# ytabatabaee/fastconsensus

Measured on AMD Instinct MI355X. Metric: consensus wall time + partition·edges/sec, LFR 1M nodes n_p=64, 1/2/4/8 GPUs, higher is better.
Workload: dtype int32

## Files before the change

fastconsensus_amd/csrc/cd_rl.hip:

```cpp
#include <hipcub/hipcub.hpp>

#include <chrono>

#include "fc_ctx.h"
#include "fc_device.h"

namespace fc {

template <class T> void exclusive_scan(Ctx& c, const T* in, T* out, int64_t n);

namespace {

constexpr int RTB = 64;
constexpr int DM = 64;
constexpr int VPWMAX = 8;
constexpr int RL_CHUNK = 16;
constexpr int RL_MAX_REPLICAS = 16384;
#ifndef FC_RL_SPLIT
#define FC_RL_SPLIT 30
#endif
#ifndef FC_LPA_TIES
#define FC_LPA_TIES 1
#endif

constexpr int32_t DONE = -1;
constexpr int NSH = 16;
constexpr int RF = 8;
constexpr double DQ_SCALE = 1099511627776.0;
constexpr int HWSLOTS = 1024;
constexpr int HTB = 256;
constexpr int HEAVY_GRID = 2048;
constexpr int SLOW_GRID = 256;
constexpr int LTB = 256;
constexpr int LPER = 8;
constexpr int NCLS = 6;
__host__ __device__ __forceinline__ int rl_class(int d) {
    return d <= 16 ? 0 : d <= 24 ? 1 : d <= 32 ? 2 : d <= 48 ? 3 : d <= DM ? 4 : 5;
}

struct RL {
    int64_t N, S, PN;
    int chunk;
    uint32_t perm_n;
    int B;
    int n_r, rbase, LG, VPW, banks, ldT;
    int lgs;
    uint32_t iter;
    uint64_t seed;
    const int64_t* rowptr;
    const int32_t* col;
    const int32_t* cw;
    const int4* vrec;
    const int64_t* kdeg;
    int64_t M2;
    int unitw;
    int wbits;
    const int32_t* colw;
    int32_t* lab;
    int32_t* tot;
    int32_t* dec;
    int64_t* slow;
    int32_t* slow_cnt;
    int4* list;
    uint64_t* lmask;
    uint64_t* vmask;
    int32_t* boff;
    int32_t* cursor;
    int32_t* voff;
    int32_t* vcursor;
    int64_t* vlist;
    uint64_t* aff;
    uint64_t* mvf;
    int32_t* active;
    int32_t* track;
    int prune, lm, track_div;
    unsigned long long* red;
    unsigned long long* sacc;
    int32_t* hscratch;
    int64_t hslots;
    double min_dq;
    int hybrid;
    const int32_t* acnt;
    int dense_div;
};
__device__ __forceinline__ bool rl_sparse(const RL& a, int r) {
    return a.hybrid && a.active[r] && a.prune && a.track[a.n_r + r] && (int64_t)a.dense_div * a.acnt[r] < a.N;
}

__device__ __forceinline__ Perm rl_perm(const RL& a, int sweep) {
    Perm P = make_perm(a.perm_n, stream_key(a.seed, SHARED_RG, a.iter, (uint32_t)sweep, 1));
    if (a.chunk) P.off = stream_key(a.seed, SHARED_RG, a.iter, (uint32_t)sweep, 3) & (RL_CHUNK - 1);
    return P;
}
__device__ __forceinline__ uint32_t rl_bucket(const RL& a, const Perm& P, uint32_t v) {
    uint32_t pos;
    if (!a.chunk) pos = perm_invert(P, v);
    else {
        const uint32_t w = v + P.off;
        pos = perm_invert(P, w / RL_CHUNK) * RL_CHUNK + w % RL_CHUNK;
    }
    return pos / (uint32_t)a.S;
}
__device__ __forceinline__ unsigned long long* rl_red(const RL& a, int r, int f) {
    return a.red + ((size_t)r * NSH + (blockIdx.x & (NSH - 1))) * RF + f;
}
__device__ __forceinline__ bool rl_better(long long s1, uint32_t h1, int32_t c1, long long s2, uint32_t h2,
                                          int32_t c2) {
    if (s1 != s2) return s1 > s2;
    if (h1 != h2) return h1 > h2;
    return c1 < c2;
}
__device__ __forceinline__ int32_t ld_off(const int32_t* base, uint32_t i) {
    return *reinterpret_cast<const int32_t*>(reinterpret_cast<const char*>(base) + (i << 2));
}
__device__ __forceinline__ int wave_max(int x) {
#pragma unroll
    for (int off = 32; off > 0; off >>= 1) x = max(x, __shfl_xor(x, off));
    return x;
}
__device__ __forceinline__ void wsync() {
    __builtin_amdgcn_wave_barrier();
    asm volatile("" ::: "memory");
}

__device__ __forceinline__ void rl_tie_flag(const RL& a, int rr, int32_t v) {
    atomicOr((unsigned long long*)&a.aff[(int64_t)(rr >> 6) * a.N + v], 1ull << (rr & 63));
}

__global__ void k_rl_init(int64_t N, int ldT, const int64_t* kdeg, int32_t* lab, int32_t* tot) {
    const int64_t i = (int64_t)blockIdx.x * blockDim.x + threadIdx.x;
    if (i >= N * ldT) return;
    const int64_t v = i / ldT;
    lab[i] = (int32_t)v;
    if (tot) tot[i] = (int32_t)kdeg[v];
}
__global__ __launch_bounds__(256) void k_rl_export(int64_t N, int n_r, int ldT, const int32_t* labT, const int32_t* sinv,
                                                   int32_t* lab) {
    __shared__ int32_t t[64][65];
    __shared__ int32_t sv[64];
    const int64_t s0 = (int64_t)blockIdx.x * 64;
    const int r0 = blockIdx.y * 64;
    const int tx = threadIdx.x & 63, ty = threadIdx.x >> 6;
    if (ty == 0) sv[tx] = s0 + tx < N ? (sinv ? sinv[s0 + tx] : (int32_t)(s0 + tx)) : -1;
    __syncthreads();
    for (int ss = ty; ss < 64; ss += 4) {
        const int32_t v = sv[ss];
        const int r = r0 + tx;
        if (v >= 0 && r < n_r) t[ss][tx] = labT[(int64_t)v * ldT + r];
    }
    __syncthreads();
    for (int rr = ty; rr < 64; rr += 4) {
        const int r = r0 + rr;
        if (r < n_r && s0 + tx < N) lab[(int64_t)r * N + s0 + tx] = t[tx][rr];
    }
}

__global__ __launch_bounds__(LTB) void k_rl_list_count(RL a, int sweep, int listed, int32_t* bcnt, int32_t* vcnt) {
    extern __shared__ unsigned long long s_dyn[];
    uint64_t* s_act = (uint64_t*)s_dyn;
    uint64_t* s_flt = s_act + a.banks;
    int* s_b = (int*)(s_flt + a.banks);
    int* s_v = s_b + a.B * NCLS;
    for (int k = threadIdx.x; k < a.B * NCLS; k += LTB) { s_b[k] = 0; s_v[k] = 0; }
    for (int b = threadIdx.x; b < a.banks; b += LTB) { s_act[b] = 0; s_flt[b] = 0; }
    __syncthreads();
    for (int r = threadIdx.x; r < a.n_r; r += LTB) {
        if (!a.active[r]) continue;
        atomicOr((unsigned long long*)&s_act[r >> 6], 1ull << (r & 63));
        if (a.prune && a.track[a.n_r + r]) atomicOr((unsigned long long*)&s_flt[r >> 6], 1ull << (r & 63));
    }
    __syncthreads();
    if (a.hybrid && listed) {
        bool any = false;
        for (int r = 0; r < a.n_r && !any; ++r) any = rl_sparse(a, r);
        if (any) return;
    }
    const Perm P = rl_perm(a, sweep);
    const int64_t v0 = (int64_t)blockIdx.x * LTB * LPER + threadIdx.x;
#pragma unroll
    for (int i = 0; i < LPER; ++i) {
        const int64_t v = v0 + (int64_t)i * LTB;
        if (v >= a.N) break;
        int nv = 0;
        for (int b = 0; b < a.banks; ++b) {
            uint64_t f = a.aff[(int64_t)b * a.N + v];
            if (listed && f) a.aff[(int64_t)b * a.N + v] = 0;
            const uint64_t m = s_act[b] & (~s_flt[b] | f);
            a.vmask[v * a.banks + b] = m;
            nv += __popcll(m);
        }
        if (nv) {
            const int sg = rl_bucket(a, P, (uint32_t)v) * NCLS + rl_class(a.vrec[v].y);
            atomicAdd(&s_b[sg], 1);
            atomicAdd(&s_v[sg], nv);
        }
    }
    __syncthreads();
    for (int k = threadIdx.x; k < a.B * NCLS; k += LTB) {
        if (s_b[k]) atomicAdd(&bcnt[k], s_b[k]);
        if (s_v[k]) atomicAdd(&vcnt[k], s_v[k]);
    }
}
__global__ void k_rl_list_plan(int nseg, int32_t* bcnt, int32_t* boff, int32_t* cursor, int32_t* vcnt,
                               int32_t* voff, int32_t* vcursor, const int32_t* n_active) {
    if (threadIdx.x != 0) return;
    int32_t acc = 0, vacc = 0;
    for (int k = 0; k < nseg; ++k) {
        boff[k] = acc; cursor[k] = acc; acc += bcnt[k];
        voff[k] = vacc; vcursor[k] = vacc; vacc += vcnt[k];
        bcnt[k] = 0; vcnt[k] = 0;
    }
    boff[nseg] = acc;
    voff[nseg] = vacc;
    voff[nseg + 1] = n_active[0];
    voff[nseg + 2] = n_active[1];
}
__global__ __launch_bounds__(LTB) void k_rl_visits_count(RL a, int64_t n_entries, int32_t* nv) {
    const int64_t e = (int64_t)blockIdx.x * LTB + threadIdx.x;
    if (e >= n_entries) return;
    int c = 0;
    for (int b = 0; b < a.banks; ++b) c += __popcll(a.lmask[e * a.banks + b]);
    nv[e] = c;
}
__global__ __launch_bounds__(LTB) void k_rl_visits_fill(RL a, int64_t n_entries, const int32_t* vpos) {
    const int64_t e = (int64_t)blockIdx.x * LTB + threadIdx.x;
    if (e >= n_entries) return;
    int64_t pos = vpos[e];
    for (int b = 0; b < a.banks; ++b) {
        uint64_t m = a.lmask[e * a.banks + b];
        while (m) {
            const int bit = __ffsll((unsigned long long)m) - 1;
            m &= m - 1;
            a.vlist[pos++] = (e << 14) | (int64_t)(b * 64 + bit);
        }
    }
}

__global__ __launch_bounds__(LTB) void k_rl_list_fill(RL a, int sweep) {
    extern __shared__ int s_lb[];
    int* s_cnt = s_lb;
    int* s_base = s_lb + a.B * NCLS;
    for (int k = threadIdx.x; k < a.B * NCLS; k += LTB) s_cnt[k] = 0;
    __syncthreads();
    const Perm P = rl_perm(a, sweep);
    int bk[LPER], loc[LPER];
    const int64_t v0 = (int64_t)blockIdx.x * LTB * LPER + threadIdx.x;
#pragma unroll
    for (int i = 0; i < LPER; ++i) {
        const int64_t v = v0 + (int64_t)i * LTB;
        bk[i] = -1;
        if (v >= a.N) continue;
        bool any = false;
        for (int b = 0; b < a.banks; ++b) any |= a.vmask[v * a.banks + b] != 0;
        if (!any) continue;
        bk[i] = (int)rl_bucket(a, P, (uint32_t)v) * NCLS + rl_class(a.vrec[v].y);
        loc[i] = atomicAdd(&s_cnt[bk[i]], 1);
    }
    __syncthreads();
    for (int k = threadIdx.x; k < a.B * NCLS; k += LTB) s_base[k] = s_cnt[k] ? atomicAdd(&a.cursor[k], s_cnt[k]) : 0;
    __syncthreads();
#pragma unroll
    for (int i = 0; i < LPER; ++i) {
        if (bk[i] < 0) continue;
        const int64_t v = v0 + (int64_t)i * LTB;
        const int64_t e = s_base[bk[i]] + loc[i];
        const int4 vr = a.vrec[v];
        a.list[e] = make_int4((int32_t)v, vr.x, vr.y, vr.z);
        for (int b = 0; b < a.banks; ++b) a.lmask[e * a.banks + b] = a.vmask[v * a.banks + b];
    }
}

struct Unit {
    int64_t e;
    int bank, s, rl, r;
    bool valid;
};
__device__ __forceinline__ Unit rl_unit(const RL& a, int64_t e0, int64_t e1, int64_t w) {
    Unit u;
    const int lane = threadIdx.x & 63;
    u.s = lane >> a.lgs;
    u.rl = lane & (a.LG - 1);
    if (a.banks == 1) { u.e = e0 + (w << (6 - a.lgs)) + u.s; u.bank = 0; }
    else { u.e = e0 + w / a.banks; u.bank = (int)(w % a.banks); }
    u.r = u.bank * 64 + u.rl;
    u.valid = u.e < e1 && u.s < a.VPW;
    return u;
}
__device__ __forceinline__ int64_t rl_items(const RL& a, int64_t n) {
    return a.banks == 1 ? (n + a.VPW - 1) / a.VPW : n * a.banks;
}

struct Hdr {
    int32_t v;
    uint64_t msk;
    int64_t rb;
    int d, kvi, ds, rr;
    bool on, heavy, work;
};
struct Rec {
    int4 e;
    uint64_t msk;
};
__device__ __forceinline__ Rec rl_fetch(const RL& a, const Unit& u) {
    Rec r;
    r.e = make_int4(-1, 0, 0, 0);
    r.msk = 0;
    if (u.valid) {
        r.e = a.list[u.e];
        r.msk = a.lmask[u.e * a.banks + u.bank];
    }
    return r;
}
__device__ __forceinline__ Hdr rl_header(const RL& a, const Unit& u, const Rec& rec) {
    Hdr h;
    h.rr = u.bank * 64 + u.rl;
    h.v = rec.e.x;
    h.msk = rec.msk;
    h.rb = (int64_t)(uint32_t)rec.e.y;
    h.d = rec.e.z;
    h.kvi = rec.e.w;
    h.on = u.valid && h.rr < a.n_r && ((h.msk >> u.rl) & 1ull);
    h.heavy = u.valid && h.d > DM;
    h.work = h.on && !h.heavy && h.d > 0;
    h.ds = (u.valid && !h.heavy && h.msk) ? h.d : 0;
    return h;
}

template <int K>
__device__ __forceinline__ void oem_sort(int32_t (&x)[K]) {
#pragma unroll
    for (int p = 1; p < K; p <<= 1)
#pragma unroll
        for (int k = p; k >= 1; k >>= 1)
#pragma unroll
            for (int j = k % p; j + k < K; j += 2 * k)
#pragma unroll
                for (int i = 0; i < k; ++i)
                    if ((i + j) / (2 * p) == (i + j + k) / (2 * p) && i + j + k < K) {
                        const int32_t a = x[i + j], b = x[i + j + k];
                        x[i + j] = min(a, b);
                        x[i + j + k] = max(a, b);
                    }
}

constexpr int WM_WIDE = 0, WM_UNIT = 1, WM_W8 = 2;
#ifndef FC_RL_SB
#define FC_RL_SB 16
#endif
constexpr int SB = FC_RL_SB;
#ifndef FC_RL_LPA_OWN
#define FC_RL_LPA_OWN 1
#endif
template <bool LOUV, int K, int WM>
__device__ __forceinline__ int32_t rl_runs(const RL& a, const Hdr& h, int sweep, int32_t (&x)[K], int32_t own,
                                           long long kown, int32_t tot_own, uint32_t home, unsigned long long& c_dq,
                                           uint32_t& c_unst, uint32_t& c_cand, bool& slow_out) {
    constexpr bool UNITW = WM == WM_UNIT;
    const uint32_t rr = (uint32_t)h.rr, ldT = (uint32_t)a.ldT;
    const int wb = UNITW ? 0 : a.wbits;
    const int32_t wm = (1 << wb) - 1;
    const bool wk = h.work;
    oem_sort<K>(x);
    int vm = INT_MIN;
    {
        int acc = 0;
        int32_t kl = (int32_t)kown;
#pragma unroll
        for (int q = 0; q < K; ++q) {
            const int32_t l = x[q] >> wb;
            const int w = UNITW ? 1 : (x[q] & wm);
            acc = (q > 0 && l == (x[q - 1] >> wb)) ? acc + w : w;
            const bool end = x[q] >= 0 && (q == K - 1 || (x[q + 1] >> wb) != l);
            vm = end ? max(vm, acc) : vm;
            if (!LOUV && !FC_RL_LPA_OWN) kl = (end && l == own) ? acc : kl;
        }
        if (!LOUV && !FC_RL_LPA_OWN) kown = kl;
        if (!LOUV && FC_RL_LPA_OWN) vm = max(vm, (int)kown);
    }
    bool hope = true;
    if (LOUV) hope = wk && ((long long)vm - kown) * a.M2 + (long long)h.kvi * ((long long)tot_own - h.kvi) > 0;
    uint32_t cm_lo = 0, cm_hi = 0;
    if (hope) {
        int acc = 0;
#pragma unroll
        for (int q = 0; q < K; ++q) {
            const int32_t l = x[q] >> wb;
            const int w = UNITW ? 1 : (x[q] & wm);
            acc = (q > 0 && l == (x[q - 1] >> wb)) ? acc + w : w;
            const bool cand = x[q] >= 0 && (q == K - 1 || (x[q + 1] >> wb) != l) && acc == vm;
            if (q < 32) cm_lo |= (uint32_t)cand << (q & 31);
            else cm_hi |= (uint32_t)cand << (q & 31);
        }
    }
    const bool own_cand = !LOUV && FC_RL_LPA_OWN && wk && kown > 0 && kown == (long long)vm;
    const int ncand = __popc(cm_lo) + __popc(cm_hi) + (own_cand ? 1 : 0);
    if (wk) c_cand += (uint32_t)ncand;
    const uint32_t tvh = hash32(stream_key(a.seed, (uint32_t)(a.rbase + h.rr), a.iter, (uint32_t)sweep, 2) ^ (uint32_t)h.v);
    int32_t dcs = -1;
    if (LOUV) {
        const long long kv = h.kvi;
        uint64_t bkey = ~0ull;
#pragma unroll
        for (int c0 = 0; c0 < K; c0 += SB) {
            const uint32_t bits = ((c0 < 32 ? cm_lo : cm_hi) >> (c0 & 31)) & ((1u << SB) - 1u);
            if (__ballot(bits != 0) == 0) continue;
            int32_t tq[SB];
#pragma unroll
            for (int i = 0; i < SB; ++i) {
                if (c0 + i >= K) break;
                const bool b = (bits >> i) & 1u;
                tq[i] = ld_off(a.tot, b ? (uint32_t)(x[c0 + i] >> wb) * ldT + rr : home);
            }
#pragma unroll
            for (int i = 0; i < SB; ++i) {
                if (c0 + i >= K) break;
                const bool b = (bits >> i) & 1u;
                const uint32_t hh = hash32(tvh ^ (uint32_t)(x[c0 + i] >> wb));
                const uint64_t key = ((uint64_t)(kv ? (uint32_t)tq[i] : 0u) << 32) | (uint32_t)~hh;
                bkey = (b && key < bkey) ? key : bkey;
            }
        }
        long long best_s = LLONG_MIN;
        uint32_t best_h = 0;
        int32_t best_c = INT_MAX;
        if (ncand != 0) {
            best_h = ~(uint32_t)bkey;
            best_c = (int32_t)(hash32_inv(best_h) ^ tvh);
            best_s = (long long)vm * a.M2 - kv * (long long)(uint32_t)(bkey >> 32);
        }
        slow_out = wk && ncand != 0 && (long long)(vm - 1) * a.M2 >= best_s;
        if (wk && ncand != 0 && !slow_out) {
            const long long G = best_s - kown * a.M2 + kv * ((long long)tot_own - kv);
            if (G > 0) {
                const double dqd = (double)G * 2.0 / ((double)a.M2 * (double)a.M2);
                c_dq += (unsigned long long)llrint(dqd * DQ_SCALE);
                dcs = best_c;
            }
        }
    } else {
        uint32_t best_h = 0;
        int32_t best_c = -1;
#pragma unroll
        for (int q = 0; q < K; ++q) {
            const bool b = ((q < 32 ? cm_lo : cm_hi) >> (q & 31)) & 1u;
            const uint32_t hh = hash32(tvh ^ (uint32_t)x[q]);
            const bool take = b && (best_c < 0 || hh > best_h);
            best_h = take ? hh : best_h;
            best_c = take ? x[q] : best_c;
        }
        if (own_cand) {
            const uint32_t hh = hash32(tvh ^ (uint32_t)own);
            if (best_c < 0 || hh > best_h) { best_h = hh; best_c = own; }
        }
        if (wk && ncand != 0) {
            c_unst += (kown != (long long)vm) ? 1 : 0;
            dcs = best_c != own ? best_c : -1;
        }
    }
    return dcs;
}

template <bool LOUV, int K, int WM>
__device__ __forceinline__ int32_t rl_sorted(const RL& a, const Hdr& h, int sweep, unsigned long long& c_dq,
                                             uint32_t& c_unst, uint32_t& c_cand, bool& slow_out) {
    constexpr bool UNITW = WM == WM_UNIT;
    slow_out = false;
    const uint32_t rr = (uint32_t)h.rr, ldT = (uint32_t)a.ldT;
    const int wb = UNITW ? 0 : a.wbits;
    const int32_t wm = (1 << wb) - 1;
    const bool wk = h.work;
    const uint32_t home = (h.v >= 0 ? (uint32_t)h.v : 0u) * ldT + rr;
    const int32_t own0 = ld_off(a.lab, home);
    const int32_t own = wk ? own0 : -1;
    const int dsw = wk ? h.ds : 0;
    int32_t x[K];
#pragma unroll
    for (int j = 0; j < K; ++j)
        x[j] = ld_off(WM == WM_W8 ? a.colw : a.col, (uint32_t)h.rb + (uint32_t)(j < dsw ? j : 0));
    int32_t tot_own = 0;
    if (LOUV) {
        const int32_t t0 = ld_off(a.tot, wk ? (uint32_t)own * ldT + rr : home);
        tot_own = wk ? t0 : 0;
    }
    long long kown = 0;
    if constexpr (UNITW) {
#pragma unroll
        for (int j = 0; j < K; ++j) {
            const int32_t lj = ld_off(a.lab, j < dsw ? (uint32_t)x[j] * ldT + rr : home);
            x[j] = j < dsw ? lj : -1;
        }
        if (LOUV || FC_RL_LPA_OWN) {
            int ko = 0;
#pragma unroll
            for (int j = 0; j < K; ++j) {
                const bool mine = x[j] == own && x[j] >= 0;
                ko += mine ? 1 : 0;
                x[j] = mine ? -1 : x[j];
            }
            kown = ko;
        }
    } else if constexpr (WM == WM_W8) {
        uint32_t wpk[(K + 3) / 4];
#pragma unroll
        for (int i = 0; i < (K + 3) / 4; ++i) wpk[i] = 0;
#pragma unroll
        for (int j = 0; j < K; ++j) wpk[j >> 2] |= (uint32_t)(x[j] & wm) << (8 * (j & 3));
#pragma unroll
        for (int j = 0; j < K; ++j) {
            const int32_t lj = ld_off(a.lab, j < dsw ? (uint32_t)(x[j] >> wb) * ldT + rr : home);
            x[j] = j < dsw ? lj : -1;
        }
        int ko = 0;
#pragma unroll
        for (int j = 0; j < K; ++j) {
            const int32_t wj = (int32_t)((wpk[j >> 2] >> (8 * (j & 3))) & 0xffu);
            const bool mine = LOUV && x[j] == own && x[j] >= 0;
            ko += mine ? wj : 0;
            x[j] = (mine || x[j] < 0) ? -1 : ((x[j] << wb) | wj);
        }
        kown = ko;
    } else {
        int32_t wv[K];
#pragma unroll
        for (int j = 0; j < K; ++j) {
            const int32_t wj = ld_off(a.cw, (uint32_t)h.rb + (uint32_t)(j < dsw ? j : 0));
            wv[j] = j < dsw ? wj : 0;
        }
#pragma unroll
        for (int j = 0; j < K; ++j) {
            const int32_t lj = ld_off(a.lab, j < dsw ? (uint32_t)x[j] * ldT + rr : home);
            x[j] = j < dsw ? lj : -1;
        }
        int ko = 0;
#pragma unroll
        for (int j = 0; j < K; ++j) {
            const bool mine = LOUV && x[j] == own && x[j] >= 0;
            ko += mine ? wv[j] : 0;
            x[j] = (mine || x[j] < 0) ? -1 : ((x[j] << wb) | wv[j]);
        }
        kown = ko;
    }
    if (LOUV) {
        const long long kvl = h.kvi;
        const bool settled = !wk || (kvl - 2 * kown) * a.M2 + kvl * ((long long)tot_own - kvl) <= 0;
        if (__ballot(!settled) == 0) return -1;
    } else if (FC_RL_LPA_OWN) {
        const bool settled = !wk || 2 * kown > (long long)dsw;
        if (__ballot(!settled) == 0) {
            if (wk) c_cand += 1u;
            return -1;
        }
    }
    constexpr int KN = (K == 32 && (FC_RL_SPLIT & 8)) ? 16 : (K == 64 && (FC_RL_SPLIT & 16)) ? 48 : K;
    if constexpr (KN < K) {
        if (__builtin_amdgcn_readfirstlane(wave_max(dsw)) <= KN) {
            int32_t y[KN];
#pragma unroll
            for (int j = 0; j < KN; ++j) y[j] = x[j];
            return rl_runs<LOUV, KN, WM>(a, h, sweep, y, own, kown, tot_own, home, c_dq, c_unst, c_cand, slow_out);
        }
    }
    return rl_runs<LOUV, K, WM>(a, h, sweep, x, own, kown, tot_own, home, c_dq, c_unst, c_cand, slow_out);
}

struct RowPre {
    int32_t col;
    int32_t w;
    int32_t own;
};
__device__ __forceinline__ Rec rl_fetch_u(const RL& a, const Unit& u) {
    Rec r = rl_fetch(a, u);
    r.e.x = __builtin_amdgcn_readfirstlane(r.e.x);
    r.e.y = __builtin_amdgcn_readfirstlane(r.e.y);
    r.e.z = __builtin_amdgcn_readfirstlane(r.e.z);
    r.e.w = __builtin_amdgcn_readfirstlane(r.e.w);
    r.msk = ((uint64_t)(uint32_t)__builtin_amdgcn_readfirstlane((int32_t)(r.msk >> 32)) << 32) |
            (uint32_t)__builtin_amdgcn_readfirstlane((int32_t)r.msk);
    return r;
}
template <int WM>
__device__ __forceinline__ RowPre rl_row_pre(const RL& a, const Unit& u, const Rec& r) {
    RowPre p;
    p.col = 0; p.w = 0; p.own = 0;
    const uint32_t lane = threadIdx.x & 63;
    if (r.e.x >= 0) {
        const int d = r.e.z;
        if (d > 0 && d <= DM) {
            const uint32_t j = lane < (uint32_t)d ? lane : 0u;
            p.col = ld_off(WM == WM_W8 ? a.colw : a.col, (uint32_t)r.e.y + j);
            if (WM == WM_WIDE) p.w = ld_off(a.cw, (uint32_t)r.e.y + j);
        }
        p.own = ld_off(a.lab, (uint32_t)r.e.x * (uint32_t)a.ldT + (uint32_t)(u.bank * 64) + lane);
    }
    return p;
}
template <bool LOUV, int K, int WM>
__device__ __forceinline__ int32_t rl_sorted_u1(const RL& a, const Hdr& h, int sweep, const RowPre& pre,
                                                unsigned long long& c_dq, uint32_t& c_unst, uint32_t& c_cand,
                                                bool& slow_out) {
    constexpr bool UNITW = WM == WM_UNIT;
    slow_out = false;
    const uint32_t rr = (uint32_t)h.rr, ldT = (uint32_t)a.ldT;
    const int wb = UNITW ? 0 : a.wbits;
    const int32_t wm = (1 << wb) - 1;
    const bool wk = h.work;
    const int ds = h.ds;
    if (ds == 0) return -1;
    const uint32_t home = (uint32_t)h.v * ldT + rr;
    const int32_t own = wk ? pre.own : -1;
    int32_t x[K];
#pragma unroll
    for (int j = 0; j < K; ++j) {
        const int32_t cj = __builtin_amdgcn_readlane(pre.col, j);
        const uint32_t id = (uint32_t)(WM == WM_W8 ? (cj >> wb) : cj);
        x[j] = ld_off(a.lab, id * ldT + rr);
    }
    int32_t tot_own = 0;
    if (LOUV) {
        const int32_t t0 = ld_off(a.tot, wk ? (uint32_t)own * ldT + rr : home);
        tot_own = wk ? t0 : 0;
    }
    long long kown = 0;
    int ko = 0;
#pragma unroll
    for (int j = 0; j < K; ++j) {
        const bool live = wk && j < ds;
        int32_t wj = 1;
        if (WM == WM_W8) wj = __builtin_amdgcn_readlane(pre.col, j) & wm;
        else if (WM == WM_WIDE) wj = __builtin_amdgcn_readlane(pre.w, j);
        const bool mine = (LOUV || FC_RL_LPA_OWN) && live && x[j] == own;
        ko += mine ? wj : 0;
        x[j] = (mine || !live) ? -1 : (UNITW ? x[j] : ((x[j] << wb) | wj));
    }
    kown = ko;
    if (LOUV) {
        const long long kvl = h.kvi;
        const bool settled = !wk || (kvl - 2 * kown) * a.M2 + kvl * ((long long)tot_own - kvl) <= 0;
        if (__ballot(!settled) == 0) return -1;
    } else if (FC_RL_LPA_OWN) {
        const bool settled = !wk || 2 * kown > (long long)ds;
        if (__ballot(!settled) == 0) {
            if (wk) c_cand += 1u;
            return -1;
        }
    }
    constexpr int KS1 = (K == 32 && (FC_RL_SPLIT & 4)) ? 16 : K;
    if constexpr (KS1 < K) {
        if (__builtin_amdgcn_readfirstlane(ds) <= KS1) {
            int32_t y[KS1];
#pragma unroll
            for (int j = 0; j < KS1; ++j) y[j] = x[j];
            return rl_runs<LOUV, KS1, WM>(a, h, sweep, y, own, kown, tot_own, home, c_dq, c_unst, c_cand, slow_out);
        }
    }
    constexpr int KS = (K == 32 && (FC_RL_SPLIT & 1)) ? 24 : (K == 64 && (FC_RL_SPLIT & 2)) ? 48 : K;
    if constexpr (KS < K) {
        if (__builtin_amdgcn_readfirstlane(ds) <= KS) {
            int32_t y[KS];
#pragma unroll
            for (int j = 0; j < KS; ++j) y[j] = x[j];
            return rl_runs<LOUV, KS, WM>(a, h, sweep, y, own, kown, tot_own, home, c_dq, c_unst, c_cand, slow_out);
        }
    }
    return rl_runs<LOUV, K, WM>(a, h, sweep, x, own, kown, tot_own, home, c_dq, c_unst, c_cand, slow_out);
}

__device__ __forceinline__ void rl_push_slow(const RL& a, bool slow, int64_t e, int rr) {
    const uint64_t m = __ballot(slow);
    if (!m) return;
    const int lane = threadIdx.x & 63;
    int base = 0;
    if (lane == 0) base = atomicAdd(a.slow_cnt, __popcll(m));
    base = __shfl(base, 0);
    if (slow) a.slow[base + __popcll(m & ((1ull << lane) - 1))] = (e << 14) | (int64_t)rr;
}

#ifndef FC_RLW16
#define FC_RLW16 1
#endif
#ifndef FC_RLW32
#define FC_RLW32 1
#endif
template <bool LOUV, int K, int WM, bool U1>
#ifndef FC_RLW32U
#define FC_RLW32U 4
#endif
#ifndef FC_RLW24U
#define FC_RLW24U 4
#endif
__global__ __launch_bounds__(RTB)
__attribute__((amdgpu_waves_per_eu(K <= 16 ? FC_RLW16 : K <= 24 ? (U1 ? FC_RLW24U : FC_RLW32) :
                                   K <= 32 ? (U1 ? FC_RLW32U : FC_RLW32) : 1)))
void k_rl_decide(RL a, int seg, int ns, int sweep) {
    const int lane = threadIdx.x & 63;
    const int64_t e0 = a.boff[seg], e1 = a.boff[seg + ns];
    const int64_t items = rl_items(a, e1 - e0);
    const int LG = a.LG;
    unsigned long long c_dq = 0;
    uint32_t c_unst = 0, c_vis = 0, c_ent = 0, c_cand = 0, c_units = 0;
    int last_r = -1;
    auto flush = [&](int r) {
        if (r < 0) return;
        for (int off = LG; off < 64; off <<= 1) {
            c_dq += __shfl_xor(c_dq, off); c_unst += __shfl_xor(c_unst, off); c_vis += __shfl_xor(c_vis, off);
            c_ent += __shfl_xor(c_ent, off); c_cand += __shfl_xor(c_cand, off); c_units += __shfl_xor(c_units, off);
        }
        if (lane < LG && r < a.n_r) {
            if (c_dq) atomicAdd(rl_red(a, r, 0), c_dq);
            if (c_unst) atomicAdd(rl_red(a, r, 1), (unsigned long long)c_unst);
            if (c_vis) atomicAdd(rl_red(a, r, 3), (unsigned long long)c_vis);
            if (c_ent) atomicAdd(rl_red(a, r, 4), (unsigned long long)c_ent);
            if (c_cand) atomicAdd(rl_red(a, r, 5), (unsigned long long)c_cand);
            if (c_units) atomicAdd(rl_red(a, r, 6), (unsigned long long)c_units);
        }
        c_dq = 0;
        c_unst = c_vis = c_ent = c_cand = c_units = 0;
    };
    Rec nxt = U1 ? rl_fetch_u(a, rl_unit(a, e0, e1, blockIdx.x)) : rl_fetch(a, rl_unit(a, e0, e1, blockIdx.x));
    Rec nx2 = nxt;
    RowPre pre;
    pre.col = pre.w = pre.own = 0;
    if constexpr (U1) {
        pre = rl_row_pre<WM>(a, rl_unit(a, e0, e1, blockIdx.x), nxt);
        nx2 = rl_fetch_u(a, rl_unit(a, e0, e1, (int64_t)blockIdx.x + gridDim.x));
    }
    for (int64_t w = blockIdx.x; w < items; w += gridDim.x) {
        const Unit u = rl_unit(a, e0, e1, w);
        if (a.banks > 1 && u.r != last_r) flush(last_r);
        last_r = a.banks > 1 ? u.r : (lane & (LG - 1));
        const Rec cur = nxt;
        RowPre pc = pre;
        if constexpr (U1) {
            nxt = nx2;
            pre = rl_row_pre<WM>(a, rl_unit(a, e0, e1, w + gridDim.x), nxt);
            nx2 = rl_fetch_u(a, rl_unit(a, e0, e1, w + 2 * (int64_t)gridDim.x));
        } else {
            nxt = rl_fetch(a, rl_unit(a, e0, e1, w + gridDim.x));
        }
        const Hdr h = rl_header(a, u, cur);
        bool slow;
        const uint32_t cc0 = c_cand;
        const int32_t dcs = U1 ? rl_sorted_u1<LOUV, K, WM>(a, h, sweep, pc, c_dq, c_unst, c_cand, slow)
                               : rl_sorted<LOUV, K, WM>(a, h, sweep, c_dq, c_unst, c_cand, slow);
        rl_push_slow(a, slow, u.e, h.rr);
        const bool tied = !LOUV && c_cand - cc0 >= 2u;
        if (!LOUV && FC_LPA_TIES) {
            const uint64_t tb = __ballot(tied && a.track[h.rr]);
            const uint64_t ts = (tb >> (u.s * LG)) & (LG == 64 ? ~0ull : ((1ull << LG) - 1ull));
            if (u.valid && u.rl == 0 && ts) atomicOr((unsigned long long*)&a.aff[(int64_t)u.bank * a.N + h.v], (unsigned long long)ts);
        }
        if (h.work) { c_vis += 1; c_ent += (uint32_t)h.d; }
        if (u.valid && u.rl == 0 && h.msk) c_units += 1;
        if (u.valid && h.rr < a.n_r) a.dec[u.e * a.ldT + h.rr] = h.work ? dcs : -1;
    }
    flush(last_r);
}

template <bool LOUV, int K, int WM>
__global__ __launch_bounds__(RTB) void k_rl_decide_v(RL a, int seg, int ns, int sweep) {
    const int64_t v0 = a.voff[seg], v1 = a.voff[seg + ns];
    for (int64_t base = (int64_t)blockIdx.x * 64; base < v1 - v0; base += (int64_t)gridDim.x * 64) {
        const int64_t i = base + (threadIdx.x & 63);
        const bool valid = i < v1 - v0;
        int64_t vp = 0;
        if (valid) vp = a.vlist[v0 + i];
        const int64_t e = vp >> 14;
        Hdr h;
        h.rr = (int)(vp & 16383);
        const int4 er = valid ? a.list[e] : make_int4(-1, 0, 0, 0);
        h.v = er.x;
        h.rb = (int64_t)(uint32_t)er.y;
        h.d = er.z;
        h.kvi = er.w;
        h.msk = 0;
        h.on = valid;
        h.heavy = false;
        h.work = valid && h.d > 0;
        h.ds = valid ? h.d : 0;
        unsigned long long c_dq = 0;
        uint32_t c_unst = 0, c_cand = 0;
        bool slow;
        const int32_t dcs = rl_sorted<LOUV, K, WM>(a, h, sweep, c_dq, c_unst, c_cand, slow);
        rl_push_slow(a, slow, e, h.rr);
        const bool tied = !LOUV && c_cand >= 2u;
        if (!LOUV && FC_LPA_TIES && valid && tied && a.track[h.rr]) rl_tie_flag(a, h.rr, h.v);
        if (valid) {
            a.dec[e * a.ldT + h.rr] = h.work ? dcs : -1;
            if (c_dq) atomicAdd(rl_red(a, h.rr, 0), c_dq);
            if (c_unst) atomicAdd(rl_red(a, h.rr, 1), (unsigned long long)c_unst);
            if (h.work) {
                atomicAdd(rl_red(a, h.rr, 3), 1ull);
                atomicAdd(rl_red(a, h.rr, 4), (unsigned long long)h.d);
            }
            if (c_cand) atomicAdd(rl_red(a, h.rr, 5), (unsigned long long)c_cand);
        }
    }
}

template <bool LOUV, int K, int WM, bool U1>
static int64_t rl_decide_slots() {
    static int64_t slots = 0;
    if (!slots) {
        int nb = 0, dev = 0;
        FC_HIP(hipOccupancyMaxActiveBlocksPerMultiprocessor(&nb, (const void*)k_rl_decide<LOUV, K, WM, U1>, RTB, 0));
        FC_HIP(hipGetDevice(&dev));
        int cus = 0;
        FC_HIP(hipDeviceGetAttribute(&cus, hipDeviceAttributeMultiprocessorCount, dev));
        slots = (int64_t)std::max(1, nb) * std::max(1, cus);
    }
    return slots;
}

struct RLShared {
    int32_t L[DM][64];
    int32_t C[VPWMAX][DM];
    int32_t W[VPWMAX][DM];
};
template <bool LOUV>
__global__ __launch_bounds__(RTB) void k_rl_decide_lds(RL a, int k, int sweep) {
    __shared__ RLShared sh;
    const int lane = threadIdx.x & 63;
    const int64_t e0 = a.boff[k * NCLS], e1 = a.boff[k * NCLS + NCLS - 1];
    const int64_t items = rl_items(a, e1 - e0);
    const int LG = a.LG, VPW = a.VPW;
    unsigned long long c_dq = 0, c_unst = 0, c_vis = 0, c_ent = 0, c_cand = 0, c_units = 0;
    int last_r = -1;
    auto flush = [&](int r) {
        if (r < 0) return;
        for (int off = LG; off < 64; off <<= 1) {
            c_dq += __shfl_xor(c_dq, off); c_unst += __shfl_xor(c_unst, off); c_vis += __shfl_xor(c_vis, off);
            c_ent += __shfl_xor(c_ent, off); c_cand += __shfl_xor(c_cand, off); c_units += __shfl_xor(c_units, off);
        }
        if (lane < LG && r < a.n_r) {
            if (c_dq) atomicAdd(rl_red(a, r, 0), c_dq);
            if (c_unst) atomicAdd(rl_red(a, r, 1), c_unst);
            if (c_vis) atomicAdd(rl_red(a, r, 3), c_vis);
            if (c_ent) atomicAdd(rl_red(a, r, 4), c_ent);
            if (c_cand) atomicAdd(rl_red(a, r, 5), c_cand);
            if (c_units) atomicAdd(rl_red(a, r, 6), c_units);
        }
        c_dq = c_unst = c_vis = c_ent = c_cand = c_units = 0;
    };
    for (int64_t w = blockIdx.x; w < items; w += gridDim.x) {
        const Unit u = rl_unit(a, e0, e1, w);
        if (a.banks > 1 && u.r != last_r) { flush(last_r); }
        last_r = a.banks > 1 ? u.r : (lane & (LG - 1));
        const int rr = u.bank * 64 + u.rl;
        int32_t v = -1;
        uint64_t msk = 0;
        int4 er = make_int4(-1, 0, 0, 0);
        if (u.valid) {
            er = a.list[u.e];
            v = er.x;
            msk = a.lmask[u.e * a.banks + u.bank];
        }
        const bool on = u.valid && rr < a.n_r && ((msk >> u.rl) & 1ull);
        const int64_t rb = (int64_t)(uint32_t)er.y;
        const int d = er.z, kvi = er.w;
        const bool heavy = u.valid && d > DM;
        const bool work = on && !heavy && d > 0;
        const int ds = (u.valid && !heavy && msk) ? d : 0;
        const int64_t lrow = (int64_t)v * a.ldT + rr;
        int32_t own = -1;
        int32_t tot_own = 0;
        if (work) own = a.lab[lrow];
        int o[VPWMAX], dsub[VPWMAX];
        int E = 0, dmax = 0;
#pragma unroll
        for (int t = 0; t < VPWMAX; ++t) {
            dsub[t] = t < VPW ? __shfl(ds, t * LG) : 0;
            o[t] = E;
            E += dsub[t];
            dmax = max(dmax, dsub[t]);
        }
        if (E == 0) {
            if (u.valid && rr < a.n_r) a.dec[u.e * a.ldT + rr] = -1;
            continue;
        }
        int64_t rbs[VPWMAX];
#pragma unroll
        for (int t = 0; t < VPWMAX; ++t) rbs[t] = t < VPW ? __shfl(rb, t * LG) : 0;
        for (int f = lane; f < E; f += 64) {
            int t = 0;
#pragma unroll
            for (int q = 1; q < VPWMAX; ++q) t += (q < VPW && f >= o[q]) ? 1 : 0;
            int64_t rbt = rbs[0];
            int ot = o[0];
#pragma unroll
            for (int q = 1; q < VPWMAX; ++q)
                if (t == q) { rbt = rbs[q]; ot = o[q]; }
            const int j = f - ot;
            sh.C[t][j] = a.col[rbt + j];
            if (!a.unitw) sh.W[t][j] = a.cw[rbt + j];
        }
        if (LOUV && work) tot_own = a.tot[(int64_t)own * a.ldT + rr];
        wsync();
        long long kown = 0;
        for (int j0 = 0; j0 < dmax; j0 += 32) {
            int32_t lb[32];
#pragma unroll
            for (int q = 0; q < 32; ++q) {
                const int j = j0 + q;
                lb[q] = (work && j < ds) ? a.lab[(int64_t)sh.C[u.s][j] * a.ldT + rr] : DONE;
            }
#pragma unroll
            for (int q = 0; q < 32; ++q) {
                const int j = j0 + q;
                if (j >= dmax) break;
                int32_t c = lb[q];
                if (LOUV && c >= 0 && c == own) {
                    kown += a.unitw ? 1 : sh.W[u.s][j];
                    c = DONE;
                }
                sh.L[j][lane] = c;
            }
        }
        wsync();
        int vm = INT_MIN, nc = 0;
        for (int j1 = 0; j1 < dmax; ++j1) {
            const int32_t c1 = sh.L[j1][lane];
            if (__ballot(c1 >= 0) == 0) continue;
            int acc = 0;
            if (c1 >= 0) {
                acc = a.unitw ? 1 : sh.W[u.s][j1];
                for (int j2 = j1 + 1; j2 < dmax; ++j2) {
                    if (sh.L[j2][lane] == c1) {
                        acc += a.unitw ? 1 : sh.W[u.s][j2];
                        sh.L[j2][lane] = DONE;
                    }
                }
                if (!LOUV && c1 == own) kown = acc;
                if (acc > vm) { vm = acc; nc = 0; }
                if (acc == vm) { sh.L[nc][lane] = c1; ++nc; }
            }
        }
        wsync();
        const uint32_t tvh = hash32(stream_key(a.seed, (uint32_t)(a.rbase + rr), a.iter, (uint32_t)sweep, 2) ^ (uint32_t)v);
        int32_t dcs = -1;
        if (LOUV) {
            long long best_s = LLONG_MIN;
            uint32_t best_h = 0;
            int32_t best_c = INT_MAX;
            const long long kv = kvi;
            const int ncm = wave_max(work ? nc : 0);
            for (int i0 = 0; i0 < ncm; i0 += 8) {
                int32_t cq[8], tq[8];
#pragma unroll
                for (int q = 0; q < 8; ++q) {
                    cq[q] = (work && i0 + q < nc) ? sh.L[i0 + q][lane] : -1;
                    tq[q] = cq[q] >= 0 ? a.tot[(int64_t)cq[q] * a.ldT + rr] : 0;
                }
#pragma unroll
                for (int q = 0; q < 8; ++q) {
                    if (cq[q] < 0) continue;
                    const long long sc = (long long)vm * a.M2 - kv * (long long)tq[q];
                    const uint32_t h = hash32(tvh ^ (uint32_t)cq[q]);
                    if (best_c == INT_MAX || rl_better(sc, h, cq[q], best_s, best_h, best_c)) {
                        best_s = sc; best_h = h; best_c = cq[q];
                    }
                }
            }
            if (work) c_cand += (unsigned long long)nc;
            const bool slow = work && nc > 0 && (long long)(vm - 1) * a.M2 >= best_s;
            if (__ballot(slow)) {
                if (slow) {
                    for (int j1 = 0; j1 < d; ++j1) {
                        const int32_t c1 = a.lab[(int64_t)a.col[rb + j1] * a.ldT + rr];
                        if (c1 == own) continue;
                        bool dup = false;
                        for (int j2 = 0; j2 < j1 && !dup; ++j2) dup = a.lab[(int64_t)a.col[rb + j2] * a.ldT + rr] == c1;
                        if (dup) continue;
                        long long val = 0;
                        for (int j2 = j1; j2 < d; ++j2)
                            if (a.lab[(int64_t)a.col[rb + j2] * a.ldT + rr] == c1) val += a.unitw ? 1 : a.cw[rb + j2];
                        if (val >= vm) continue;
                        const long long sc = val * a.M2 - kv * (long long)a.tot[(int64_t)c1 * a.ldT + rr];
                        const uint32_t h = hash32(tvh ^ (uint32_t)c1);
                        ++c_cand;
                        if (rl_better(sc, h, c1, best_s, best_h, best_c)) { best_s = sc; best_h = h; best_c = c1; }
                    }
                }
            }
            if (work && nc > 0) {
                const long long G = best_s - kown * a.M2 + kv * ((long long)tot_own - kv);
                if (G > 0) {
                    const double dqd = (double)G * 2.0 / ((double)a.M2 * (double)a.M2);
                    c_dq += (unsigned long long)llrint(dqd * DQ_SCALE);
                    dcs = best_c;
                }
            }
        } else {
            uint32_t best_h = 0;
            int32_t best_c = -1;
            for (int i = 0; i < nc; ++i) {
                const int32_t c = sh.L[i][lane];
                const uint32_t h = hash32(tvh ^ (uint32_t)c);
                if (best_c < 0 || h > best_h) { best_h = h; best_c = c; }
            }
            if (work) {
                c_cand += (unsigned long long)nc;
                if (nc > 0) {
                    c_unst += (kown != (long long)vm) ? 1 : 0;
                    dcs = best_c != own ? best_c : -1;
                }
                if (FC_LPA_TIES && nc >= 2 && a.track[rr]) rl_tie_flag(a, rr, v);
            }
        }
        if (work) { c_vis += 1; c_ent += (unsigned long long)d; }
        if (u.valid && u.rl == 0 && msk && !heavy) c_units += 1;
        if (u.valid && rr < a.n_r) a.dec[u.e * a.ldT + rr] = work ? dcs : -1;
        wsync();
    }
    flush(last_r);
}

template <bool LOUV>
__global__ __launch_bounds__(HTB) void k_rl_exact(RL a, int k, int sweep) {
    __shared__ int32_t key[HTB / 64][HWSLOTS], val[HTB / 64][HWSLOTS];
    const int lane = threadIdx.x & 63, wv = threadIdx.x >> 6;
    const int64_t h0 = a.boff[k * NCLS + NCLS - 1], h1 = a.boff[k * NCLS + NCLS];
    const int64_t ch = (h1 - h0) * a.n_r;
    const int64_t cnt = ch + (LOUV ? *a.slow_cnt : 0);
    const int64_t gw = (int64_t)blockIdx.x * (HTB / 64) + wv, nw = (int64_t)gridDim.x * (HTB / 64);
    for (int64_t item = gw; item < cnt; item += nw) {
        int64_t e;
        int rr;
        const bool heavy = item < ch;
        if (heavy) {
            e = h0 + item / a.n_r;
            rr = (int)(item % a.n_r);
            const uint64_t msk = a.lmask[e * a.banks + (rr >> 6)];
            if (!((msk >> (rr & 63)) & 1ull)) continue;
        } else {
            const int64_t p = a.slow[item - ch];
            e = p >> 14;
            rr = (int)(p & 16383);
        }
        const int32_t v = a.list[e].x;
        const int64_t rb = a.rowptr[v], d = a.rowptr[v + 1] - rb;
        uint32_t slots = 64;
        while (slots < 2 * (uint32_t)d) slots <<= 1;
        int32_t* keys = key[wv];
        int32_t* vals = val[wv];
        if (slots > HWSLOTS) {
            slots = (uint32_t)a.hslots;
            keys = a.hscratch + gw * 2 * a.hslots;
            vals = keys + slots;
        }
        for (uint32_t q = lane; q < slots; q += 64) { keys[q] = -1; vals[q] = 0; }
        wsync();
        for (int64_t j = rb + lane; j < rb + d; j += 64) {
            const int32_t c = a.lab[(int64_t)a.col[j] * a.ldT + rr];
            const int32_t w = a.unitw ? 1 : a.cw[j];
            uint32_t h = hash32((uint32_t)c) & (slots - 1);
            while (true) {
                const int32_t prev = atomicCAS(&keys[h], -1, c);
// ... 628 lines not shown
```

Measured before the change: 21.57 billion.

## Reduce register pressure in U1 row-local decide kernel with scheduling fences

Adds sched_barrier fences and asm register pins inside the odd-even merge sort and run scans of the U1 path, and batches label gathers in groups so the compiler cannot hoist every load at once. The U1 loop is rewritten to walk (edge, bank) coordinates incrementally instead of recomputing units per item. Cold kernel arguments are reloaded from the kernarg segment only when needed, and rarely-taken tie and slow paths are skipped with ballots. A waves-per-EU hint is added for K=64 U1. The aim is lower VGPR use and fewer spills, at the cost of possibly less instruction-level parallelism.

```diff
diff --git a/fastconsensus_amd/csrc/cd_rl.hip b/fastconsensus_amd/csrc/cd_rl.hip
--- a/fastconsensus_amd/csrc/cd_rl.hip
+++ b/fastconsensus_amd/csrc/cd_rl.hip
@@ -326,8 +326,12 @@
     return h;
 }
 
-template <int K>
+#ifndef FC_RL_OEM_FENCE
+#define FC_RL_OEM_FENCE 8
+#endif
+template <int K, bool FENCED>
 __device__ __forceinline__ void oem_sort(int32_t (&x)[K]) {
+    int n = 0;
 #pragma unroll
     for (int p = 1; p < K; p <<= 1)
 #pragma unroll
@@ -340,6 +344,8 @@
                         const int32_t a = x[i + j], b = x[i + j + k];
                         x[i + j] = min(a, b);
                         x[i + j + k] = max(a, b);
+                        if (FENCED && FC_RL_OEM_FENCE && ++n % (FC_RL_OEM_FENCE ? FC_RL_OEM_FENCE : 1) == 0)
+                            __builtin_amdgcn_sched_barrier(0);
                     }
 }
 
@@ -347,11 +353,13 @@
 #ifndef FC_RL_SB
 #define FC_RL_SB 16
 #endif
-constexpr int SB = FC_RL_SB;
+#ifndef FC_RL_SB64
+#define FC_RL_SB64 FC_RL_SB
+#endif
 #ifndef FC_RL_LPA_OWN
 #define FC_RL_LPA_OWN 1
 #endif
-template <bool LOUV, int K, int WM>
+template <bool LOUV, int K, int WM, bool TIGHT>
 __device__ __forceinline__ int32_t rl_runs(const RL& a, const Hdr& h, int sweep, int32_t (&x)[K], int32_t own,
                                            long long kown, int32_t tot_own, uint32_t home, unsigned long long& c_dq,
                                            uint32_t& c_unst, uint32_t& c_cand, bool& slow_out) {
@@ -360,7 +368,8 @@
     const int wb = UNITW ? 0 : a.wbits;
     const int32_t wm = (1 << wb) - 1;
     const bool wk = h.work;
-    oem_sort<K>(x);
+    oem_sort<K, TIGHT>(x);
+    if (TIGHT && FC_RL_OEM_FENCE) __builtin_amdgcn_sched_barrier(0);
     int vm = INT_MIN;
     {
         int acc = 0;
@@ -373,6 +382,7 @@
             const bool end = x[q] >= 0 && (q == K - 1 || (x[q + 1] >> wb) != l);
             vm = end ? max(vm, acc) : vm;
             if (!LOUV && !FC_RL_LPA_OWN) kl = (end && l == own) ? acc : kl;
+            if (TIGHT && FC_RL_OEM_FENCE && (q & 7) == 7) __builtin_amdgcn_sched_barrier(0);
         }
         if (!LOUV && !FC_RL_LPA_OWN) kown = kl;
         if (!LOUV && FC_RL_LPA_OWN) vm = max(vm, (int)kown);
@@ -381,6 +391,9 @@
     if (LOUV) hope = wk && ((long long)vm - kown) * a.M2 + (long long)h.kvi * ((long long)tot_own - h.kvi) > 0;
     uint32_t cm_lo = 0, cm_hi = 0;
     if (hope) {
+#pragma unroll
+        for (int q = 0; q < K; ++q)
+            if (TIGHT) asm volatile("" : "+v"(x[q]));
         int acc = 0;
 #pragma unroll
         for (int q = 0; q < K; ++q) {
@@ -388,8 +401,11 @@
             const int w = UNITW ? 1 : (x[q] & wm);
             acc = (q > 0 && l == (x[q - 1] >> wb)) ? acc + w : w;
             const bool cand = x[q] >= 0 && (q == K - 1 || (x[q + 1] >> wb) != l) && acc == vm;
-            if (q < 32) cm_lo |= (uint32_t)cand << (q & 31);
-            else cm_hi |= (uint32_t)cand << (q & 31);
+            uint32_t cb = cand ? 1u : 0u;
+            if (TIGHT) asm volatile("" : "+v"(cb));
+            if (q < 32) cm_lo |= cb << (q & 31);
+            else cm_hi |= cb << (q & 31);
+            if (TIGHT && FC_RL_OEM_FENCE && (q & 7) == 7) __builtin_amdgcn_sched_barrier(0);
         }
     }
     const bool own_cand = !LOUV && FC_RL_LPA_OWN && wk && kown > 0 && kown == (long long)vm;
@@ -400,6 +416,7 @@
     if (LOUV) {
         const long long kv = h.kvi;
         uint64_t bkey = ~0ull;
+        constexpr int SB = K == 64 ? FC_RL_SB64 : FC_RL_SB;
 #pragma unroll
         for (int c0 = 0; c0 < K; c0 += SB) {
             const uint32_t bits = ((c0 < 32 ? cm_lo : cm_hi) >> (c0 & 31)) & ((1u << SB) - 1u);
@@ -458,6 +475,11 @@
         }
     }
     return dcs;
+}
+
+__device__ __forceinline__ int32_t rl_own_key(int32_t k) {
+    asm volatile("" : "+v"(k));
+    return k;
 }
 
 template <bool LOUV, int K, int WM>
@@ -557,12 +579,16 @@
             int32_t y[KN];
 #pragma unroll
             for (int j = 0; j < KN; ++j) y[j] = x[j];
-            return rl_runs<LOUV, KN, WM>(a, h, sweep, y, own, kown, tot_own, home, c_dq, c_unst, c_cand, slow_out);
-        }
-    }
-    return rl_runs<LOUV, K, WM>(a, h, sweep, x, own, kown, tot_own, home, c_dq, c_unst, c_cand, slow_out);
-}
-
+            return rl_runs<LOUV, KN, WM, false>(a, h, sweep, y, own, kown, tot_own, home, c_dq, c_unst, c_cand, slow_out);
+        }
+    }
+    return rl_runs<LOUV, K, WM, false>(a, h, sweep, x, own, kown, tot_own, home, c_dq, c_unst, c_cand, slow_out);
+}
+
+#ifndef FC_RL_BC
+#define FC_RL_BC 16
+#endif
+constexpr int RL_BC = FC_RL_BC;
 struct RowPre {
     int32_t col;
     int32_t w;
@@ -610,10 +636,14 @@
     const int32_t own = wk ? pre.own : -1;
     int32_t x[K];
 #pragma unroll
-    for (int j = 0; j < K; ++j) {
-        const int32_t cj = __builtin_amdgcn_readlane(pre.col, j);
-        const uint32_t id = (uint32_t)(WM == WM_W8 ? (cj >> wb) : cj);
-        x[j] = ld_off(a.lab, id * ldT + rr);
+    for (int j0 = 0; j0 < K; j0 += RL_BC) {
+#pragma unroll
+        for (int j = j0; j < j0 + RL_BC && j < K; ++j) {
+            const int32_t cj = __builtin_amdgcn_readlane(pre.col, j);
+            const uint32_t id = (uint32_t)(WM == WM_W8 ? (cj >> wb) : cj);
+            x[j] = ld_off(a.lab, id * ldT + rr);
+        }
+        __builtin_amdgcn_sched_barrier(0);
     }
     int32_t tot_own = 0;
     if (LOUV) {
@@ -631,6 +661,7 @@
         const bool mine = (LOUV || FC_RL_LPA_OWN) && live && x[j] == own;
         ko += mine ? wj : 0;
         x[j] = (mine || !live) ? -1 : (UNITW ? x[j] : ((x[j] << wb) | wj));
+        asm volatile("" : "+v"(x[j]));
     }
     kown = ko;
     if (LOUV) {
@@ -649,8 +680,8 @@
         if (__builtin_amdgcn_readfirstlane(ds) <= KS1) {
             int32_t y[KS1];
 #pragma unroll
-            for (int j = 0; j < KS1; ++j) y[j] = x[j];
-            return rl_runs<LOUV, KS1, WM>(a, h, sweep, y, own, kown, tot_own, home, c_dq, c_unst, c_cand, slow_out);
+            for (int j = 0; j < KS1; ++j) y[j] = rl_own_key(x[j]);
+            return rl_runs<LOUV, KS1, WM, true>(a, h, sweep, y, own, kown, tot_own, home, c_dq, c_unst, c_cand, slow_out);
         }
     }
     constexpr int KS = (K == 32 && (FC_RL_SPLIT & 1)) ? 24 : (K == 64 && (FC_RL_SPLIT & 2)) ? 48 : K;
@@ -658,11 +689,11 @@
         if (__builtin_amdgcn_readfirstlane(ds) <= KS) {
             int32_t y[KS];
 #pragma unroll
-            for (int j = 0; j < KS; ++j) y[j] = x[j];
-            return rl_runs<LOUV, KS, WM>(a, h, sweep, y, own, kown, tot_own, home, c_dq, c_unst, c_cand, slow_out);
-        }
-    }
-    return rl_runs<LOUV, K, WM>(a, h, sweep, x, own, kown, tot_own, home, c_dq, c_unst, c_cand, slow_out);
+            for (int j = 0; j < KS; ++j) y[j] = rl_own_key(x[j]);
+            return rl_runs<LOUV, KS, WM, true>(a, h, sweep, y, own, kown, tot_own, home, c_dq, c_unst, c_cand, slow_out);
+        }
+    }
+    return rl_runs<LOUV, K, WM, true>(a, h, sweep, x, own, kown, tot_own, home, c_dq, c_unst, c_cand, slow_out);
 }
 
 __device__ __forceinline__ void rl_push_slow(const RL& a, bool slow, int64_t e, int rr) {
@@ -673,6 +704,12 @@
     if (lane == 0) base = atomicAdd(a.slow_cnt, __popcll(m));
     base = __shfl(base, 0);
     if (slow) a.slow[base + __popcll(m & ((1ull << lane) - 1))] = (e << 14) | (int64_t)rr;
+}
+
+__device__ __forceinline__ const RL& rl_cold() {
+    auto p = __builtin_amdgcn_kernarg_segment_ptr();
+    asm volatile("" : "+s"(p));
+    return *(const RL*)p;
 }
 
 #ifndef FC_RLW16
@@ -688,14 +725,19 @@
 #ifndef FC_RLW24U
 #define FC_RLW24U 4
 #endif
+#ifndef FC_RLW64U
+#define FC_RLW64U 1
+#endif
+#ifndef FC_RLW64U_UNIT
+#define FC_RLW64U_UNIT 1
+#endif
 __global__ __launch_bounds__(RTB)
 __attribute__((amdgpu_waves_per_eu(K <= 16 ? FC_RLW16 : K <= 24 ? (U1 ? FC_RLW24U : FC_RLW32) :
-                                   K <= 32 ? (U1 ? FC_RLW32U : FC_RLW32) : 1)))
+                                   K <= 32 ? (U1 ? FC_RLW32U : FC_RLW32) : (K == 64 && U1) ? (WM == WM_W8 ? FC_RLW64U : FC_RLW64U_UNIT) : 1)))
 void k_rl_decide(RL a, int seg, int ns, int sweep) {
     const int lane = threadIdx.x & 63;
     const int64_t e0 = a.boff[seg], e1 = a.boff[seg + ns];
-    const int64_t items = rl_items(a, e1 - e0);
-    const int LG = a.LG;
+    const int LG = U1 ? 64 : a.LG;
     unsigned long long c_dq = 0;
     uint32_t c_unst = 0, c_vis = 0, c_ent = 0, c_cand = 0, c_units = 0;
     int last_r = -1;
@@ -705,53 +747,85 @@
             c_dq += __shfl_xor(c_dq, off); c_unst += __shfl_xor(c_unst, off); c_vis += __shfl_xor(c_vis, off);
             c_ent += __shfl_xor(c_ent, off); c_cand += __shfl_xor(c_cand, off); c_units += __shfl_xor(c_units, off);
         }
-        if (lane < LG && r < a.n_r) {
-            if (c_dq) atomicAdd(rl_red(a, r, 0), c_dq);
-            if (c_unst) atomicAdd(rl_red(a, r, 1), (unsigned long long)c_unst);
-            if (c_vis) atomicAdd(rl_red(a, r, 3), (unsigned long long)c_vis);
-            if (c_ent) atomicAdd(rl_red(a, r, 4), (unsigned long long)c_ent);
-            if (c_cand) atomicAdd(rl_red(a, r, 5), (unsigned long long)c_cand);
-            if (c_units) atomicAdd(rl_red(a, r, 6), (unsigned long long)c_units);
+        const RL& cold = U1 ? rl_cold() : a;
+        if (lane < LG && r < cold.n_r) {
+            if (c_dq) atomicAdd(rl_red(cold, r, 0), c_dq);
+            if (c_unst) atomicAdd(rl_red(cold, r, 1), (unsigned long long)c_unst);
+            if (c_vis) atomicAdd(rl_red(cold, r, 3), (unsigned long long)c_vis);
+            if (c_ent) atomicAdd(rl_red(cold, r, 4), (unsigned long long)c_ent);
+            if (c_cand) atomicAdd(rl_red(cold, r, 5), (unsigned long long)c_cand);
+            if (c_units) atomicAdd(rl_red(cold, r, 6), (unsigned long long)c_units);
         }
         c_dq = 0;
         c_unst = c_vis = c_ent = c_cand = c_units = 0;
     };
-    Rec nxt = U1 ? rl_fetch_u(a, rl_unit(a, e0, e1, blockIdx.x)) : rl_fetch(a, rl_unit(a, e0, e1, blockIdx.x));
-    Rec nx2 = nxt;
-    RowPre pre;
-    pre.col = pre.w = pre.own = 0;
-    if constexpr (U1) {
-        pre = rl_row_pre<WM>(a, rl_unit(a, e0, e1, blockIdx.x), nxt);
-        nx2 = rl_fetch_u(a, rl_unit(a, e0, e1, (int64_t)blockIdx.x + gridDim.x));
-    }
-    for (int64_t w = blockIdx.x; w < items; w += gridDim.x) {
-        const Unit u = rl_unit(a, e0, e1, w);
-        if (a.banks > 1 && u.r != last_r) flush(last_r);
-        last_r = a.banks > 1 ? u.r : (lane & (LG - 1));
-        const Rec cur = nxt;
-        RowPre pc = pre;
-        if constexpr (U1) {
-            nxt = nx2;
-            pre = rl_row_pre<WM>(a, rl_unit(a, e0, e1, w + gridDim.x), nxt);
-            nx2 = rl_fetch_u(a, rl_unit(a, e0, e1, w + 2 * (int64_t)gridDim.x));
-        } else {
-            nxt = rl_fetch(a, rl_unit(a, e0, e1, w + gridDim.x));
-        }
-        const Hdr h = rl_header(a, u, cur);
-        bool slow;
-        const uint32_t cc0 = c_cand;
-        const int32_t dcs = U1 ? rl_sorted_u1<LOUV, K, WM>(a, h, sweep, pc, c_dq, c_unst, c_cand, slow)
-                               : rl_sorted<LOUV, K, WM>(a, h, sweep, c_dq, c_unst, c_cand, slow);
-        rl_push_slow(a, slow, u.e, h.rr);
+    auto finish = [&](const Unit& u, const Hdr& h, int32_t dcs, bool slow, uint32_t cc0) {
+        if (!U1) rl_push_slow(a, slow, u.e, h.rr);
+        else if (__ballot(slow)) rl_push_slow(rl_cold(), slow, u.e, h.rr);
         const bool tied = !LOUV && c_cand - cc0 >= 2u;
-        if (!LOUV && FC_LPA_TIES) {
-            const uint64_t tb = __ballot(tied && a.track[h.rr]);
+        if (!LOUV && FC_LPA_TIES && (!U1 || __ballot(tied))) {
+            const RL& cold = U1 ? rl_cold() : a;
+            const uint64_t tb = __ballot(tied && cold.track[h.rr]);
             const uint64_t ts = (tb >> (u.s * LG)) & (LG == 64 ? ~0ull : ((1ull << LG) - 1ull));
-            if (u.valid && u.rl == 0 && ts) atomicOr((unsigned long long*)&a.aff[(int64_t)u.bank * a.N + h.v], (unsigned long long)ts);
+            if (u.valid && u.rl == 0 && ts) atomicOr((unsigned long long*)&cold.aff[(int64_t)u.bank * cold.N + h.v], (unsigned long long)ts);
         }
         if (h.work) { c_vis += 1; c_ent += (uint32_t)h.d; }
         if (u.valid && u.rl == 0 && h.msk) c_units += 1;
         if (u.valid && h.rr < a.n_r) a.dec[u.e * a.ldT + h.rr] = h.work ? dcs : -1;
+    };
+    if constexpr (U1) {
+        const int banks = a.banks;
+        const uint32_t ge = gridDim.x / (uint32_t)banks, gb = gridDim.x % (uint32_t)banks;
+        auto unit_of = [&](int64_t e, int bank) {
+            Unit u;
+            u.e = e; u.bank = bank; u.s = 0; u.rl = lane; u.r = bank * 64 + lane;
+            u.valid = e < e1;
+            return u;
+        };
+        auto step = [&](int64_t& e, int& bank) {
+            e += ge; bank += (int)gb;
+            if (bank >= banks) { bank -= banks; ++e; }
+        };
+        int64_t en = e0 + blockIdx.x / (uint32_t)banks;
+        int bn = (int)(blockIdx.x % (uint32_t)banks);
+        Rec nxt = rl_fetch_u(a, unit_of(en, bn));
+        RowPre pre = rl_row_pre<WM>(a, unit_of(en, bn), nxt);
+        int64_t e2 = en;
+        int b2 = bn;
+        step(e2, b2);
+        Rec nx2 = rl_fetch_u(a, unit_of(e2, b2));
+        while (en < e1) {
+            const Unit u = unit_of(en, bn);
+            if (banks > 1 && u.r != last_r) flush(last_r);
+            last_r = banks > 1 ? u.r : lane;
+            const Rec cur = nxt;
+            const RowPre pc = pre;
+            en = e2; bn = b2;
+            nxt = nx2;
+            pre = rl_row_pre<WM>(a, unit_of(en, bn), nxt);
+            step(e2, b2);
+            nx2 = rl_fetch_u(a, unit_of(e2, b2));
+            const Hdr h = rl_header(a, u, cur);
+            bool slow;
+            const uint32_t cc0 = c_cand;
+            const int32_t dcs = rl_sorted_u1<LOUV, K, WM>(a, h, sweep, pc, c_dq, c_unst, c_cand, slow);
+            finish(u, h, dcs, slow, cc0);
+        }
+    } else {
+        const int64_t items = rl_items(a, e1 - e0);
+        Rec nxt = rl_fetch(a, rl_unit(a, e0, e1, blockIdx.x));
+        for (int64_t w = blockIdx.x; w < items; w += gridDim.x) {
+            const Unit u = rl_unit(a, e0, e1, w);
+            if (a.banks > 1 && u.r != last_r) flush(last_r);
+            last_r = a.banks > 1 ? u.r : (lane & (LG - 1));
+            const Rec cur = nxt;
+            nxt = rl_fetch(a, rl_unit(a, e0, e1, w + gridDim.x));
+            const Hdr h = rl_header(a, u, cur);
+            bool slow;
+            const uint32_t cc0 = c_cand;
+            const int32_t dcs = rl_sorted<LOUV, K, WM>(a, h, sweep, c_dq, c_unst, c_cand, slow);
+            finish(u, h, dcs, slow, cc0);
+        }
     }
     flush(last_r);
 }
```

After: 21.84 billion (median of 6 runs). 1.2% higher.
